# CyrilMorel42/LZ4-JPEG

Measured on AMD Instinct MI355X. Metric: LZ4 compress GB/s + JPEG DCT Mpixel/s at 1/2/4/8 MI355X; % HBM roofline, higher is better.
Workload: dtype u8

## Files before the change

include/lz4r.h:

```cpp
#ifndef LZ4R_H
#define LZ4R_H

#include <stddef.h>
#include <stdint.h>

#ifdef __cplusplus
extern "C" {
#endif

#define LZ4R_BLOCK 300
#define LZ4R_BLOCK_BOUND 1152

#define LZ4R_OK 0
#define LZ4R_ERR_ARG (-1)
#define LZ4R_ERR_TOO_SMALL (-2)
#define LZ4R_ERR_CAPACITY (-3)
#define LZ4R_ERR_HIP (-4)
#define LZ4R_ERR_NOMEM (-5)
#define LZ4R_ERR_CORRUPT (-6)
#define LZ4R_LEN_CORRUPT (1ull << 63)


typedef struct lz4r_ctx lz4r_ctx;

int lz4r_ctx_create(lz4r_ctx **ctx);
void lz4r_ctx_destroy(lz4r_ctx *ctx);

size_t lz4r_compress_bound(size_t n);
size_t lz4r_nblocks(size_t n);

size_t lz4r_launch_chunk_blocks(void);

int lz4r_compress_device(lz4r_ctx *ctx, const void *d_in, size_t n,
                         void *d_out, size_t cap, size_t *out_len,
                         void *stream);

int lz4r_compress_async(lz4r_ctx *ctx, const void *d_in, size_t n,
                        void *d_out, size_t cap, void *d_out_len,
                        void *stream);

int lz4r_compress_segment_async(lz4r_ctx *ctx, const void *d_in, size_t n,
                                void *d_out, size_t cap, void *d_out_len,
                                int final_shard, void *stream);

int lz4r_block_matches_device(const void *d_in, size_t n, void *d_matches, void *stream);

int lz4r_window_matches_device(const void *d_in, size_t n, void *d_matches, void *stream);

int lz4r_copy_block_sizes(const lz4r_ctx *ctx, void *dst, size_t count,
                          void *stream);

int lz4r_copy_block_offsets(const lz4r_ctx *ctx, void *dst, size_t count,
                            void *stream);

int lz4r_block_offsets_device(const lz4r_ctx *ctx, const void **d_offsets,
                              size_t *count);

int lz4r_decompress(const uint8_t *in, size_t in_len, uint8_t *out, size_t cap,
                    size_t *out_len);

int lz4r_decompress_device(const void *d_in, size_t in_len, const void *d_block_offsets,
                           size_t nb, void *d_out, size_t out_cap, void *d_result,
                           void *stream);

int lz4r_decompress_stream_device(const void *d_in, size_t in_len, void *d_out,
                                  size_t out_cap, size_t *out_len, void *stream);

int lz4r_decompress_stream(const uint8_t *in, size_t in_len, uint8_t *out, size_t cap,
                           size_t *out_len);

typedef struct lz4r_read { uint64_t src, len, dst; } lz4r_read;

size_t lz4r_read_items(size_t max_len);

int lz4r_read_device(const void *d_in, size_t in_len, const void *d_block_offsets,
                     size_t nb, const void *d_reads, size_t nreads, size_t max_len,
                     void *d_out, size_t out_cap, void *d_result, void *stream);

int lz4r_stream_index_device(const void *d_in, size_t in_len, void *d_block_offsets,
                             size_t cap_blocks, size_t *nb, size_t *decoded_len, void *stream);

int lz4r_compress(const uint8_t *in, size_t n, uint8_t *out, size_t cap,
                  size_t *out_len);

int lz4r_check(lz4r_ctx *ctx, void *stream);

int lz4r_set_timing(lz4r_ctx *ctx, int enable);
int lz4r_last_timing(lz4r_ctx *ctx, float *ms_call, float *ms_match);
int lz4r_timed_calls(lz4r_ctx *ctx, size_t max, float *ms_call, float *ms_match, size_t *count);

const char *lz4r_strerror(int code);

#ifdef __cplusplus
}
#endif
#endif
```

lz4-jpeg_amd/csrc/lz4r.hip:

```cpp
#include <hip/hip_ext.h>
#include <hip/hip_runtime.h>
#include <limits.h>
#include <stdint.h>
#include <stdio.h>
#include <stdlib.h>
#include <algorithm>
#include <new>
#include <vector>

#include "../../include/lz4r.h"
#include "lz4r_prof.h"
#include "wave64.h"
#include "lz4r_layout.h"
#include "lz4r_tiles.h"
#include "lz4r_matches.h"
#include "lz4r_scan.h"
#include "lz4r_emit.h"

#ifndef LZ4R_CHUNK_LOG2
#define LZ4R_CHUNK_LOG2 24
#endif
constexpr size_t kChunk = size_t(1) << LZ4R_CHUNK_LOG2;
static_assert(kChunk % kPart == 0, "chunks start on a scan partial");
static_assert((kChunk / 8) * 8 * 64 < (size_t(1) << 32), "chunk grid fits HIP's limit");
constexpr size_t kMaxInput = size_t(1) << 40;

struct lz4r_ctx {
  int device = 0;
  size_t cap_blocks = 0;
  size_t cap_slots = 0;
  uint16_t *bsizes = nullptr;
  uint64_t *boff = nullptr;
  uint8_t *slots = nullptr;
  uint32_t *tsz = nullptr;
  uint32_t *gsum = nullptr;
  uint64_t *part = nullptr;
  uint64_t *len = nullptr;
  uint32_t *status = nullptr;
  uint64_t *verdict = nullptr;
  size_t last_nb = 0;
  bool checkable = false;
  struct timed_set {
    hipEvent_t a = nullptr, c = nullptr;
    std::vector<hipEvent_t> tiles;
    size_t chunks = 0;
  };
  std::vector<timed_set> tsets;
  size_t timed_calls = 0;
  bool timing = false;
};
constexpr size_t kTimedCalls = 4096;

namespace {

void free_scratch(lz4r_ctx *c) {
  (void)hipFree(c->bsizes);
  (void)hipFree(c->boff);
  (void)hipFree(c->tsz);
  (void)hipFree(c->gsum);
  (void)hipFree(c->part);
  (void)hipFree(c->slots);
  c->bsizes = nullptr;
  c->boff = nullptr;
  c->slots = nullptr;
  c->tsz = nullptr;
  c->gsum = nullptr;
  c->part = nullptr;
  c->cap_blocks = 0;
  c->cap_slots = 0;
}

int ensure_scratch(lz4r_ctx *c, size_t nb) {
  const size_t need_slots = std::min(nb, kChunk);
  if (nb <= c->cap_blocks && need_slots <= c->cap_slots) return LZ4R_OK;
  free_scratch(c);
  const size_t cap = nb + nb / 8 + 1024;
  const size_t cap_slots = std::min(cap, kChunk);
  const size_t parts = (cap + kPart - 1) / kPart;
  const size_t groups = (cap + kGT - 1) / kGT;
  if (hipMalloc(&c->slots, cap_slots * (size_t)kSlot) != hipSuccess ||
      hipMalloc(&c->bsizes, cap * sizeof(uint16_t)) != hipSuccess ||
      hipMalloc(&c->boff, cap * sizeof(uint64_t)) != hipSuccess ||
      hipMalloc(&c->tsz, cap * sizeof(uint32_t)) != hipSuccess ||
      hipMalloc(&c->gsum, groups * sizeof(uint32_t)) != hipSuccess ||
      hipMalloc(&c->part, parts * sizeof(uint64_t)) != hipSuccess) {
    (void)hipGetLastError();
    free_scratch(c);
    return LZ4R_ERR_NOMEM;
  }
  c->cap_blocks = cap;
  c->cap_slots = cap_slots;
  return LZ4R_OK;
}

int make_event(hipEvent_t *e) {
  return hipEventCreateWithFlags(e, hipEventDisableSystemFence) == hipSuccess ? LZ4R_OK
                                                                               : LZ4R_ERR_HIP;
}

int next_timed_set(lz4r_ctx *c, size_t nchunks, lz4r_ctx::timed_set **out) {
  const size_t i = c->timed_calls % kTimedCalls;
  if (c->tsets.size() <= i) c->tsets.resize(i + 1);
  lz4r_ctx::timed_set &t = c->tsets[i];
  if ((!t.a && make_event(&t.a) != LZ4R_OK) || (!t.c && make_event(&t.c) != LZ4R_OK))
    return LZ4R_ERR_HIP;
  while (t.tiles.size() < 2 * nchunks) {
    hipEvent_t e = nullptr;
    if (make_event(&e) != LZ4R_OK) return LZ4R_ERR_HIP;
    t.tiles.push_back(e);
  }
  t.chunks = nchunks;
  *out = &t;
  return LZ4R_OK;
}

void destroy_events(lz4r_ctx *c) {
  for (auto &t : c->tsets) {
    if (t.a) (void)hipEventDestroy(t.a);
    if (t.c) (void)hipEventDestroy(t.c);
    for (hipEvent_t e : t.tiles) (void)hipEventDestroy(e);
  }
  c->tsets.clear();
}

int timed_ms(const lz4r_ctx::timed_set &t, float *ms_call, float *ms_match) {
  if (hipEventSynchronize(t.c) != hipSuccess) return LZ4R_ERR_HIP;
  float a = 0.f, b = 0.f;
  if (hipEventElapsedTime(&a, t.a, t.c) != hipSuccess) return LZ4R_ERR_HIP;
  for (size_t k = 0; k < t.chunks; ++k) {
    float x = 0.f;
    if (hipEventElapsedTime(&x, k == 0 ? t.a : t.tiles[2 * k], t.tiles[2 * k + 1]) != hipSuccess)
      return LZ4R_ERR_HIP;
    b += x;
  }
  *ms_call = a;
  *ms_match = b;
  return LZ4R_OK;
}

int run(lz4r_ctx *c, const void *d_in, size_t n, void *d_out, size_t cap,
        void *d_len, int hdr, void *stream) {
  if (!c || !d_in || !d_out || !d_len) return LZ4R_ERR_ARG;
  if (hdr && n < (size_t)kBlk) return LZ4R_ERR_TOO_SMALL;
  if (n == 0 || n > kMaxInput) return LZ4R_ERR_ARG;
  const size_t nb = (n + kBlk - 1) / kBlk;
  const size_t nchunks = (nb + kChunk - 1) / kChunk;
  int rc = ensure_scratch(c, nb);
  if (rc != LZ4R_OK) return rc;
  hipStream_t s = static_cast<hipStream_t>(stream);
  const bool timed = c->timing;
  lz4r_ctx::timed_set *ts = nullptr;
  if (timed && (rc = next_timed_set(c, nchunks, &ts)) != LZ4R_OK) return rc;
  auto ev = [&](hipEvent_t e) { return timed ? e : nullptr; };
  const uint8_t *in = static_cast<const uint8_t *>(d_in);
  uint8_t *const ovfs = c->slots + c->cap_slots * (size_t)kHead;
  for (size_t k = 0; k < nchunks; ++k) {
    const size_t b0 = k * kChunk;
    const size_t nbc = std::min(kChunk, nb - b0);
    const size_t b1 = b0 + nbc;
    const uint32_t last_n = (uint32_t)(b1 == nb ? n - (nb - 1) * kBlk : kBlk);
    const uint32_t runs = (uint32_t)((nbc + 8 * kTileRun - 1) / (8 * kTileRun));
    const uint32_t per = runs * kTileRun;
    hipEvent_t t0 = timed ? (k == 0 ? ts->a : ts->tiles[2 * k]) : nullptr;
    hipEvent_t t1 = timed ? ts->tiles[2 * k + 1] : nullptr;
    const auto tiles = ((uintptr_t)in & 3) == 0 ? lz4_tiles<true> : lz4_tiles<false>;
    hipExtLaunchKernelGGL(tiles, dim3(8 * runs), dim3(64), 0, s, t0, t1, 0u, in + b0 * kBlk,
                          (uint32_t)nbc, per, last_n, c->slots, ovfs, c->tsz + b0,
                          c->bsizes + b0, c->status);
    const size_t p0 = b0 / kPart, np = (nbc + kPart - 1) / kPart;
    hipLaunchKernelGGL(lz4_scan_reduce, dim3((unsigned)np), dim3(256), 0, s, c->tsz, b1, p0,
                       c->gsum, c->part);
    hipLaunchKernelGGL(lz4_scan_partials, dim3(1), dim3(1024), 0, s, c->part + p0, np,
                       (uint64_t)hdr, k == 0 ? 1 : 0, k + 1 == nchunks ? 1 : 0, c->status,
                       static_cast<uint64_t *>(d_len), c->verdict);
    const size_t g0 = b0 / kGT, ng = (nbc + kGT - 1) / kGT;
    hipExtLaunchKernelGGL(lz4_emit, dim3((unsigned)(8 * ((ng * kGSplit + 7) / 8))), dim3(64 * kEW), 0, s, nullptr,
                          k + 1 == nchunks ? ev(ts ? ts->c : nullptr) : nullptr, 0u, in,
                          (const uint8_t *)c->slots, (const uint8_t *)ovfs, b0,
                          (const uint32_t *)c->tsz, b1, g0, (const uint32_t *)c->gsum,
                          (const uint64_t *)c->part, static_cast<uint8_t *>(d_out), (uint64_t)cap,
                          hdr, (uint64_t)nb, (uint32_t)(n - (nb - 1) * kBlk), c->boff);
  }
  if (timed) ++c->timed_calls;
  c->last_nb = nb;
  c->checkable = true;
  const hipError_t e = hipGetLastError();
  if (e != hipSuccess && getenv("LZ4R_DEBUG"))
    fprintf(stderr, "lz4r: %s\n", hipGetErrorString(e));
  return e == hipSuccess ? LZ4R_OK : LZ4R_ERR_HIP;
}

int copy_per_block(const lz4r_ctx *c, const void *src, size_t elem, void *dst, size_t count,
                   void *stream) {
  if (!dst || count > c->last_nb) return LZ4R_ERR_ARG;
  if (count == 0) return LZ4R_OK;
  hipStream_t s = static_cast<hipStream_t>(stream);
  if (hipMemcpyAsync(dst, src, count * elem, hipMemcpyDefault, s) != hipSuccess ||
      hipStreamSynchronize(s) != hipSuccess)
    return LZ4R_ERR_HIP;
  return LZ4R_OK;
}

}

extern "C" {

int lz4r_ctx_create(lz4r_ctx **out) {
  if (!out) return LZ4R_ERR_ARG;
  lz4r_ctx *c = new (std::nothrow) lz4r_ctx();
  if (!c) return LZ4R_ERR_NOMEM;
  if (hipGetDevice(&c->device) != hipSuccess ||
      hipMalloc(&c->len, 3 * sizeof(uint64_t)) != hipSuccess ||
      hipMemset(c->len, 0, 3 * sizeof(uint64_t)) != hipSuccess) {
    lz4r_ctx_destroy(c);
    return LZ4R_ERR_HIP;
  }
  c->status = reinterpret_cast<uint32_t *>(c->len + 1);
  c->verdict = c->len + 2;
  *out = c;
  return LZ4R_OK;
}

void lz4r_ctx_destroy(lz4r_ctx *c) {
  if (!c) return;
  free_scratch(c);
  (void)hipFree(c->len);
  destroy_events(c);
  delete c;
}

size_t lz4r_nblocks(size_t n) { return (n + kBlk - 1) / kBlk; }

size_t lz4r_launch_chunk_blocks(void) { return kChunk; }

size_t lz4r_compress_bound(size_t n) { return 1 + lz4r_nblocks(n) * (size_t)LZ4R_BLOCK_BOUND; }

int lz4r_compress_async(lz4r_ctx *c, const void *d_in, size_t n, void *d_out, size_t cap,
                        void *d_len, void *stream) {
  return run(c, d_in, n, d_out, cap, d_len, 1, stream);
}

int lz4r_compress_segment_async(lz4r_ctx *c, const void *d_in, size_t n, void *d_out,
                                size_t cap, void *d_len, int final_shard, void *stream) {
  if (!c || !d_len) return LZ4R_ERR_ARG;
  if (!final_shard && n % kBlk != 0) return LZ4R_ERR_ARG;
  if (n == 0) {
    c->last_nb = 0;
    c->checkable = false;
    hipStream_t s = static_cast<hipStream_t>(stream);
    if (c->timing) {
      lz4r_ctx::timed_set *ts = nullptr;
      const int rc = next_timed_set(c, 0, &ts);
      if (rc != LZ4R_OK) return rc;
      (void)hipEventRecord(ts->a, s);
      (void)hipEventRecord(ts->c, s);
      ++c->timed_calls;
    }
    return hipMemsetAsync(d_len, 0, sizeof(uint64_t), s) == hipSuccess ? LZ4R_OK : LZ4R_ERR_HIP;
  }
  return run(c, d_in, n, d_out, cap, d_len, 0, stream);
}

int lz4r_compress_device(lz4r_ctx *c, const void *d_in, size_t n, void *d_out, size_t cap,
                         size_t *out_len, void *stream) {
  if (!c || !out_len) return LZ4R_ERR_ARG;
  int rc = run(c, d_in, n, d_out, cap, c->len, 1, stream);
  if (rc != LZ4R_OK) return rc;
  uint64_t got = 0;
  hipStream_t s = static_cast<hipStream_t>(stream);
  hipError_t e = hipMemcpyAsync(&got, c->len, sizeof(got), hipMemcpyDeviceToHost, s);
  if (e == hipSuccess) e = hipStreamSynchronize(s);
  if (e != hipSuccess) {
    if (getenv("LZ4R_DEBUG")) fprintf(stderr, "lz4r: %s\n", hipGetErrorString(e));
    return LZ4R_ERR_HIP;
  }
  *out_len = (size_t)(got & ~kLenCorrupt);
  if (got & kLenCorrupt) return LZ4R_ERR_CORRUPT;
  return *out_len > cap ? LZ4R_ERR_CAPACITY : LZ4R_OK;
}

int lz4r_block_matches_device(const void *d_in, size_t n, void *d_matches, void *stream) {
  if (!d_in || !d_matches || n == 0 || n > kMaxInput) return LZ4R_ERR_ARG;
  const size_t nb = (n + kBlk - 1) / kBlk;
  const uint8_t *in = static_cast<const uint8_t *>(d_in);
  uint32_t *mo = static_cast<uint32_t *>(d_matches);
  for (size_t b0 = 0; b0 < nb; b0 += kChunk) {
    const size_t nbc = std::min(kChunk, nb - b0);
    const uint32_t last_n = (uint32_t)(b0 + nbc == nb ? n - (nb - 1) * kBlk : kBlk);
    hipLaunchKernelGGL(lz4_matches, dim3((unsigned)nbc), dim3(64), 0,
                       static_cast<hipStream_t>(stream), in + b0 * kBlk, (uint32_t)nbc, last_n,
                       mo + b0 * kBlk);
  }
  return hipGetLastError() == hipSuccess ? LZ4R_OK : LZ4R_ERR_HIP;
}

int lz4r_window_matches_device(const void *d_in, size_t n, void *d_matches, void *stream) {
  if (!d_in || !d_matches || n == 0 || n > 0xFFFFFFFFull) return LZ4R_ERR_ARG;
  constexpr size_t kPosChunk = size_t(1) << 26;
  for (size_t p0 = 0; p0 < n; p0 += kPosChunk) {
    const size_t np = std::min(kPosChunk, n - p0);
    hipLaunchKernelGGL(lz4_window_matches, dim3((unsigned)((np + 3) / 4)), dim3(256), 0,
                       static_cast<hipStream_t>(stream), static_cast<const uint8_t *>(d_in),
                       (uint32_t)n, (uint32_t)p0, static_cast<uint32_t *>(d_matches));
  }
  return hipGetLastError() == hipSuccess ? LZ4R_OK : LZ4R_ERR_HIP;
}

int lz4r_copy_block_sizes(const lz4r_ctx *c, void *dst, size_t count, void *stream) {
  if (!c) return LZ4R_ERR_ARG;
  return copy_per_block(c, c->bsizes, sizeof(uint16_t), dst, count, stream);
}

int lz4r_copy_block_offsets(const lz4r_ctx *c, void *dst, size_t count, void *stream) {
  if (!c) return LZ4R_ERR_ARG;
  return copy_per_block(c, c->boff, sizeof(uint64_t), dst, count, stream);
}

int lz4r_block_offsets_device(const lz4r_ctx *c, const void **d_offsets, size_t *count) {
  if (!c || !d_offsets || !count) return LZ4R_ERR_ARG;
  *d_offsets = c->boff;
  *count = c->last_nb;
  return LZ4R_OK;
}

int lz4r_compress(const uint8_t *in, size_t n, uint8_t *out, size_t cap, size_t *out_len) {
  if (!in || !out || !out_len) return LZ4R_ERR_ARG;
  if (n < (size_t)kBlk) return LZ4R_ERR_TOO_SMALL;
  lz4r_ctx *c = nullptr;
  int rc = lz4r_ctx_create(&c);
  if (rc != LZ4R_OK) return rc;
  void *din = nullptr, *dout = nullptr;
  const size_t dcap = lz4r_compress_bound(n);
  if (hipMalloc(&din, n + 16) != hipSuccess || hipMalloc(&dout, dcap) != hipSuccess) {
    (void)hipFree(din);
    lz4r_ctx_destroy(c);
    return LZ4R_ERR_NOMEM;
  }
  if (hipMemcpy(din, in, n, hipMemcpyHostToDevice) != hipSuccess) rc = LZ4R_ERR_HIP;
  size_t got = 0;
  if (rc == LZ4R_OK) rc = lz4r_compress_device(c, din, n, dout, dcap, &got, nullptr);
  if (rc == LZ4R_OK) {
    *out_len = got;
    if (got > cap) rc = LZ4R_ERR_CAPACITY;
    else if (hipMemcpy(out, dout, got, hipMemcpyDeviceToHost) != hipSuccess) rc = LZ4R_ERR_HIP;
  }
  (void)hipFree(din);
  (void)hipFree(dout);
  lz4r_ctx_destroy(c);
  return rc;
}

int lz4r_check(lz4r_ctx *c, void *stream) {
  if (!c) return LZ4R_ERR_ARG;
  if (!c->checkable) return LZ4R_OK;
  uint64_t v = 0;
  hipStream_t s = static_cast<hipStream_t>(stream);
  if (hipMemcpyAsync(&v, c->verdict, sizeof(v), hipMemcpyDeviceToHost, s) != hipSuccess ||
      hipStreamSynchronize(s) != hipSuccess)
    return LZ4R_ERR_HIP;
  return v ? LZ4R_ERR_CORRUPT : LZ4R_OK;
}

int lz4r_set_timing(lz4r_ctx *c, int enable) {
  if (!c) return LZ4R_ERR_ARG;
  c->timing = enable != 0;
  if (c->timing) c->timed_calls = 0;
  return LZ4R_OK;
}

int lz4r_last_timing(lz4r_ctx *c, float *ms_call, float *ms_match) {
  if (!c || c->timed_calls == 0) return LZ4R_ERR_ARG;
  float a = 0.f, b = 0.f;
  const int rc = timed_ms(c->tsets[(c->timed_calls - 1) % kTimedCalls], &a, &b);
  if (rc != LZ4R_OK) return rc;
  if (ms_call) *ms_call = a;
  if (ms_match) *ms_match = b;
  return LZ4R_OK;
}

int lz4r_timed_calls(lz4r_ctx *c, size_t max, float *ms_call, float *ms_match, size_t *count) {
  if (!c || !count || (max && (!ms_call || !ms_match))) return LZ4R_ERR_ARG;
  const size_t n = std::min(std::min(c->timed_calls, kTimedCalls), max);
  for (size_t j = 0; j < n; ++j) {
    const size_t i = (c->timed_calls - n + j) % kTimedCalls;
    const int rc = timed_ms(c->tsets[i], &ms_call[j], &ms_match[j]);
    if (rc != LZ4R_OK) return rc;
  }
  *count = n;
  return LZ4R_OK;
}

const char *lz4r_strerror(int code) {
  switch (code) {
    case LZ4R_OK: return "ok";
    case LZ4R_ERR_ARG: return "invalid argument";
    case LZ4R_ERR_TOO_SMALL: return "input shorter than one 300-byte block";
    case LZ4R_ERR_CAPACITY: return "output buffer too small";
    case LZ4R_ERR_HIP: return "HIP runtime error";
    case LZ4R_ERR_NOMEM: return "device allocation failed";
    case LZ4R_ERR_CORRUPT: return "corrupt stream";
    default: return "unknown error";
  }
}

}
```

lz4-jpeg_amd/csrc/lz4r_tiles.h:

```cpp
#pragma once
#include <type_traits>

#include "lz4r_prof.h"
#include "lz4r_tile_lds.h"

namespace {

typedef unsigned int u32x2 __attribute__((ext_vector_type(2)));
typedef unsigned int u32x3 __attribute__((ext_vector_type(3)));
struct TileKeys {
  u32x2 r0;
  u32x3 r[4];
};

__device__ __forceinline__ int block_lane() {
  int lane = threadIdx.x;
  asm volatile("" : "+v"(lane));
  __builtin_assume(lane >= 0 && lane < 64);
  return lane;
}

__device__ __forceinline__ void load_keys(TileKeys &K, const uint8_t *__restrict__ src, int lane) {
  typedef u32x2 u32x2_a4 __attribute__((aligned(4)));
  typedef u32x3 u32x3_a4 __attribute__((aligned(4)));
  const uint32_t *bw = reinterpret_cast<const uint32_t *>(src) + (lane >> 2);
  K.r0 = *reinterpret_cast<const u32x2_a4 *>(bw);
#pragma unroll
  for (int r = 1; r < 5; ++r) K.r[r - 1] = *reinterpret_cast<const u32x3_a4 *>(bw + 16 * r - 1);
}

__device__ __forceinline__ void keys_arrived(TileKeys &K) {
  asm volatile("" : "+v"(K.r0), "+v"(K.r[0]), "+v"(K.r[1]), "+v"(K.r[2]), "+v"(K.r[3]));
}

struct RecBatch {
  uint32_t seqv = 0;
  uint32_t p0 = 0;
};
constexpr int kHalf = 32;

__device__ __forceinline__ uint32_t half_incl_add(uint32_t v) {
  v += dpp<0x111, 0xf, 0xf>(v);
  v += dpp<0x112, 0xf, 0xf>(v);
  v += dpp<0x114, 0xf, 0xf>(v);
  v += dpp<0x118, 0xf, 0xf>(v);
  v += dpp<0x142, 0xa, 0xf>(v);
  return v;
}

__device__ __forceinline__ void store_block_totals(uint64_t m, uint32_t tb, int lane, uint32_t hdr,
                                                   uint32_t w, uint8_t *heads, uint32_t *usz,
                                                   uint16_t *bsizes) {
  const uint32_t bl = tb + (uint32_t)lane;
  uint64_t save;
  asm volatile(
      "s_and_saveexec_b64 %0, %1\n\t"
      "global_store_dword %2, %5, %7\n\t"
      "global_store_dword %3, %6, %8\n\t"
      "global_store_short %4, %6, %9\n\t"
      "s_or_b64 exec, exec, %0"
      : "=&s"(save)
      : "s"(m), "v"(bl * (uint32_t)kHead), "v"(bl * 4u), "v"(bl * 2u), "v"(hdr), "v"(w), "s"(heads),
        "s"(usz), "s"(bsizes)
      : "memory", "scc");
}

template <bool kFast>
__device__ __forceinline__ void flush_records(const uint32_t wv, const uint32_t f0,
                                              const uint32_t f1, const uint32_t tb,
                                              uint8_t *__restrict__ heads,
                                              uint8_t *__restrict__ ovfs,
                                              uint32_t *__restrict__ usz,
                                              uint16_t *__restrict__ bsizes, const int lane) {
  constexpr int n = kBlk;
  const int M = (int)((wv >> 9) & 255u);
  const int end = (int)(wv >> 19);
  const uint32_t cq = (uint32_t)(end - M);
  const uint32_t upv = dpp<0x138, 0xf, 0xf>((uint32_t)end);
  const int pend = (int)sel_mask(0x0000000100000001ull, 0u, upv);
  const int L = (int)cq - pend;
  const uint64_t am = (((1ull << f0) - 1ull) | ((1ull << f1) - 1ull) << kHalf) & ballot(pend < n);
  uint32_t ws;
  if constexpr (kFast) {
    ws = (uint32_t)(L + 5) + (L >= 15 ? 1u : 0u) + (L == 270 ? 1u : 0u) + (M >= 19 ? 1u : 0u);
  } else {
    ws = (uint32_t)(L + 5 + (L >= 15 ? 1 : 0) + (L == 270 ? 1 : 0)) * 0x10001u;
    ws += M >= 19 ? 0x10001u : 0u;
    ws += (uint32_t)(M - 1) < 3u ? 0x10000u : 0u;
  }
  const uint32_t sc = half_incl_add(sel_mask(am, ws, 0u));
  const uint32_t t0 = (uint32_t)__builtin_amdgcn_readlane((int)sc, kHalf - 1);
  const uint32_t t1 = lane63(sc);
  const uint32_t ns0 = (uint32_t)__popc((uint32_t)am), ns1 = (uint32_t)__popc((uint32_t)(am >> kHalf));
  uint32_t hdr, wb;
  if constexpr (kFast) {
    hdr = write_lane<0>(t1 | (ns1 << 16), t0 | (ns0 << 16));
    wb = (hdr & 0xFFFFu) + 3u;
  } else {
    uint32_t z0 = t0 >> 16, z1 = t1 >> 16;
    asm("" : "+s"(z0));
    asm("" : "+s"(z1));
    hdr = write_lane<0>(z1 | (ns1 << 16), z0 | (ns0 << 16));
    wb = write_lane<0>((t1 & 0xFFFFu) + 3u, (t0 & 0xFFFFu) + 3u);
  }
  constexpr uint64_t kHeadLanes = ((1ull << (kHeadW - 1)) - 1ull) * 0x0000000100000001ull;
  const uint32_t x4 = 4u * (uint32_t)lane, h32 = (uint32_t)lane & (uint32_t)kHalf;
  store_lanes1(am & kHeadLanes, reinterpret_cast<uint32_t *>(heads + (size_t)tb * kHead),
               x4 - h32 * ((128 - kHead) / kHalf), wv);
  const uint64_t om = am & ~kHeadLanes;
  if (om)
    store_lanes1(om, reinterpret_cast<uint32_t *>(ovfs + (size_t)tb * kOvf) - kHeadW,
                 x4 + (h32 << 3) + (h32 >> 1), wv);
  static_assert(kOvf - 4 * kHalf == 8 * kHalf + kHalf / 2, "the second overflow slot from lane & 32");
  store_block_totals(f1 ? 3ull : 1ull, tb, lane, hdr, wb, heads, usz, bsizes);
}
static_assert((128 - kHead) % kHalf == 0 && kHeadW - 1 < kHalf, "the second half's records");

template <bool kMatchesOnly, bool kFull>
__device__ __forceinline__ void encode_block(TileLds &S, int n_arg, const uint8_t *__restrict__ gsrc,
                                            TileKeys &K, const uint8_t *__restrict__ next,
                                            uint32_t *__restrict__ mout,
                                            uint8_t *__restrict__ heads,
                                            uint8_t *__restrict__ ovfs,
                                            uint32_t *__restrict__ status, const int lane,
                                            ProfClock &prof, RecBatch &B, const bool flush_after,
                                            uint32_t *__restrict__ usz,
                                            uint16_t *__restrict__ bsizes, const uint32_t t) {
  const int n = kFull ? kBlk : n_arg;
  constexpr int base = kInOff;

  const int nk = n >= 4 ? n - 3 : 0;

  bool walk[5];
  uint32_t qn = 0;
  uint32_t key[5];
  {
    const uint32_t sh = (uint32_t)lane & 3u;
    const uint32_t *bw = reinterpret_cast<const uint32_t *>(S.buf) + (kInOff >> 2) + (lane >> 2);
    uint32_t pt[5], adr[5], set[5];
    const uint32_t dummy = (uint32_t)(kRecOff + 4 * (192 + lane) - kHeadOff);
#pragma unroll
    for (int r = 0; r < 5; ++r) {
      const uint32_t w1 = !kFull ? bw[16 * r] : r ? K.r[r ? r - 1 : 0].y : K.r0.x;
      const uint32_t w2 = !kFull ? bw[16 * r + 1] : r ? K.r[r ? r - 1 : 0].z : K.r0.y;
      key[r] = __builtin_amdgcn_alignbyte(w2, w1, sh);
      const uint32_t hv = key[r] * 2654435761u;
      if (r == 0) {
        const uint32_t pb = (uint32_t)__builtin_amdgcn_update_dpp(0, (int)key[0], 0x138, 0xf,
                                                                 0xf, false);
        pt[0] = __builtin_amdgcn_perm(pb, key[0], 0x00040C0Cu);
      } else {
        const uint32_t w0 = kFull ? K.r[r - 1].x : bw[16 * r - 1];
        pt[r] = __builtin_amdgcn_perm(w1, w0, 0x04030C0Cu + sh * 0x01010000u);
      }
      const int p = 64 * r + lane;
      const bool act = (kFull && r < 4) || p < nk;
// ... 164 lines not shown

  PROF_MARK(4);
  const uint32_t lim = (uint32_t)(4 * n + 1) << 17;
  auto walk_words = [&](uint32_t &sq, int l0) {
    int l1 = l0;
    if (w0 < lim) {
      static_assert(kWordOff < 65536, "ds_read offset field");
      uint32_t w = w0, va = w0 >> 17, vt;
      asm volatile(
          "s_mov_b32 m0, %7\n"
          "1:\n\t"
          "v_writelane_b32 %0, %1, m0\n\t"
          "ds_read_b32 %3, %2 offset:%c6\n\t"
          "s_add_u32 m0, m0, 1\n\t"
          "s_waitcnt lgkmcnt(0)\n\t"
          "v_readfirstlane_b32 %1, %3\n\t"
          "v_lshrrev_b32 %2, 17, %3\n\t"
          "s_cmp_lt_u32 %1, %5\n\t"
          "s_cbranch_scc1 1b\n\t"
          "s_mov_b32 %4, m0"
          : "+v"(sq), "+s"(w), "+v"(va), "=&v"(vt), "=&s"(l1)
          : "s"(lim), "i"(kWordOff), "s"(l0)
          : "scc", "memory");
    }
    return l1;
  };
  constexpr bool kBat = kFull && kTileRun > 1;
  int it;
  uint32_t seqv;
  if constexpr (kBat) {
    const uint32_t p0 = B.p0;
    const int l0 = (int)(p0 >> 16);
    const uint32_t before = B.seqv;
    seqv = before;
    __builtin_amdgcn_s_setprio(3);
    const int l1 = walk_words(seqv, l0);
    __builtin_amdgcn_s_setprio(0);
    it = l1 - l0;
    const bool fits = it < kHalf;
    PROF_MARK(5);
    keys_arrived(K);
    PROF_MARK(7);
    uint32_t f0 = p0 & 255u, f1 = 0u, slowm = p0 & 256u, rv = before;
    if (fits) {
      rv = (lane == l1) ? (uint32_t)n << 19 : seqv;
      slowm |= fastw ? 0u : 256u;
      if (l0 == 0) {
        if (!flush_after) {
          B.seqv = rv;
          B.p0 = (uint32_t)(it + 1) | slowm | (uint32_t)kHalf << 16;
          return;
        }
        f0 = (uint32_t)(it + 1);
      } else {
        f1 = (uint32_t)(it + 1);
      }
    }
    B.p0 = 0;
    if (f0) {
      const uint32_t tb = t - (uint32_t)(l0 >> 5);
      if (slowm == 0u)
        flush_records<true>(rv, f0, f1, tb, heads, ovfs, usz, bsizes, lane);
      else
        flush_records<false>(rv, f0, f1, tb, heads, ovfs, usz, bsizes, lane);
    }
    PROF_MARK(6);
    if (fits) return;
    seqv = 0;
    walk_words(seqv, 0);
  } else {
    seqv = 0;
    __builtin_amdgcn_s_setprio(3);
    it = walk_words(seqv, 0);
    __builtin_amdgcn_s_setprio(0);
  }
  const bool slow = it > 64;
  int Sv_slow = 0;
  if (slow) {
    const uint8_t *const wb = reinterpret_cast<const uint8_t *>(S.word);
    for (uint32_t w = w0; w < lim;
         w = (uint32_t)__builtin_amdgcn_readfirstlane(
             (int)*reinterpret_cast<const uint32_t *>(wb + (w >> 17)))) {
      if (lane == 0) S.seq()[Sv_slow] = w;
      ++Sv_slow;
    }
    wave_sync();
  }
  PROF_MARK(5);
  uint32_t *const head = reinterpret_cast<uint32_t *>(heads + (size_t)t * kHead);
  uint32_t *const ovf = reinterpret_cast<uint32_t *>(ovfs + (size_t)t * kOvf);
  int nseq = 0;
  int ocar = 3;
  int szsum = 0;
  int end_prev = 0;
  auto round = [&](auto fast, int s0, uint32_t wv) {
    const int kk = s0 + lane;
    const int M = (int)((wv >> 9) & 255u);
    const int end = (int)(wv >> 19);
    const uint32_t cq = (uint32_t)(end - M);
    const uint64_t ismm = ballot((int)cq < n);
    const int nm_r = __popcll(ismm);
    const uint32_t upv = dpp<0x138, 0xf, 0xf>((uint32_t)end);
    const int pend = lane == 0 ? end_prev : (int)upv;
    end_prev = (int)lane63((uint32_t)end);
    const int L = (int)cq - pend;
    const uint64_t am = ismm | (ballot(lane == nm_r) & ballot(pend < n));
    if constexpr (decltype(fast)::value) {
      const uint32_t ws = (uint32_t)(L + 5) + (L >= 15 ? 1u : 0u) + (L == 270 ? 1u : 0u) +
                          (M >= 19 ? 1u : 0u);
      const uint32_t tot = lane63(wave_incl_add(sel_mask(am, ws, 0u)));
      ocar += (int)tot;
      szsum += (int)tot;
    } else {
      uint32_t ws = (uint32_t)(L + 5 + (L >= 15 ? 1 : 0) + (L == 270 ? 1 : 0)) * 0x10001u;
      ws += M >= 19 ? 0x10001u : 0u;
      ws += (uint32_t)(M - 1) < 3u ? 0x10000u : 0u;
      const uint32_t tot = lane63(wave_incl_add(sel_mask(am, ws, 0u)));
      ocar += (int)(tot & 0xFFFFu);
      szsum += (int)(tot >> 16);
    }
    if (s0 == 0) {
      store_lanes1(am & ((1ull << (kHeadW - 1)) - 1), head, 4u * (uint32_t)kk, wv);
      if (am >> (kHeadW - 1)) store_lanes1(am >> (kHeadW - 1) << (kHeadW - 1), ovf - kHeadW,
                                           4u * (uint32_t)kk, wv);
    } else {
      store_lanes1(am, ovf - kHeadW, 4u * (uint32_t)kk, wv);
    }
    nseq += (int)__popcll(am);
    return nm_r == 64;
  };
  {
    const uint32_t wtail = (uint32_t)n << 19;
    const uint32_t c0 = slow ? S.seq()[lane] : (lane < it ? seqv : wtail);
    auto rounds = [&](auto fast) {
      if (round(fast, 0, c0)) {
        for (int s0 = 64;; s0 += 64) {
          const int kk = s0 + lane;
          if (!round(fast, s0, slow && kk < Sv_slow ? S.seq()[kk] : wtail)) break;
        }
      }
    };
    if (fastw)
      rounds(std::true_type{});
    else
      rounds(std::false_type{});
  }
  PROF_MARK(6);
  store_block_totals(1ull, t, lane, (uint32_t)szsum | ((uint32_t)nseq << 16), (uint32_t)ocar, heads,
                     usz, bsizes);
}

template <bool kAligned>
__global__ __launch_bounds__(64) __attribute__((amdgpu_waves_per_eu(8, 8))) void lz4_tiles(
    const uint8_t *__restrict__ in, uint32_t nb, uint32_t per, uint32_t last_n,
    uint8_t *__restrict__ heads, uint8_t *__restrict__ ovfs, uint32_t *__restrict__ usz,
    uint16_t *__restrict__ bsizes, uint32_t *__restrict__ status) {
  __shared__ TileLds S;
  ProfClock prof = PROF_START();
  const uint32_t t0 = (blockIdx.x & 7u) * per + (blockIdx.x >> 3) * (uint32_t)kTileRun;
  if (t0 >= nb) return;
  const uint32_t t1 = kTileRun == 1 ? t0 + 1 : min(t0 + (uint32_t)kTileRun, nb);
  const uint32_t nbg = nb + (last_n >= 24 ? 1u : 0u);
  auto full = [&](uint32_t t) { return kAligned && t + 2 < nbg; };
  TileKeys K;
  RecBatch B;
  const uint8_t *src = in + (size_t)t0 * kBlk;
  for (uint32_t t = t0; t < t1; ++t, src += kBlk) {
    const int lane = block_lane();
    const int n = t + 1 + (last_n >= 24 ? 1u : 0u) == nbg ? (int)last_n : kBlk;
    if (full(t)) {
      if (t == t0) {
        load_keys(K, src, lane);
        keys_arrived(K);
        PROF_MARK(7);
      }
      const bool pf = kTileRun > 1 && t + 1 < t1 && full(t + 1);
      encode_block<false, true>(S, kBlk, src, K, pf ? src + kBlk : src, nullptr, heads, ovfs,
                                status, lane, prof, B, !pf, usz, bsizes, t);
    } else {
      for (int i = lane; i < n; i += 64) S.buf[kInOff + i] = src[i];
      if (lane < 16) S.buf[kInOff + n + lane] = 0;
      wave_sync();
      if (t == t0) PROF_MARK(7);
      encode_block<false, false>(S, n, nullptr, K, nullptr, nullptr, heads, ovfs, status, lane,
                                 prof, B, true, usz, bsizes, t);
    }
    wave_sync();
  }
  PROF_FLUSH();
}

}
```

lz4-jpeg_amd/lz4jpeg/_lib.py:

```python
import ctypes
import os

_HERE = os.path.dirname(os.path.abspath(__file__))
LIB_PATH = os.environ.get("LZ4JPEG_LIB") or os.path.join(_HERE, "liblz4jpeg.so")

_c_size = ctypes.c_size_t
_vp = ctypes.c_void_p
_i = ctypes.c_int

SIGNATURES = [
    ("lz4r_ctx_create", _i, [ctypes.POINTER(_vp)]),
    ("lz4r_ctx_destroy", None, [_vp]),
    ("lz4r_compress_bound", _c_size, [_c_size]),
    ("lz4r_nblocks", _c_size, [_c_size]),
    ("lz4r_launch_chunk_blocks", _c_size, []),
    ("lz4r_compress_device", _i, [_vp, _vp, _c_size, _vp, _c_size, ctypes.POINTER(_c_size), _vp]),
    ("lz4r_compress_async", _i, [_vp, _vp, _c_size, _vp, _c_size, _vp, _vp]),
    ("lz4r_compress_segment_async", _i, [_vp, _vp, _c_size, _vp, _c_size, _vp, _i, _vp]),
    ("lz4r_copy_block_sizes", _i, [_vp, _vp, _c_size, _vp]),
    ("lz4r_copy_block_offsets", _i, [_vp, _vp, _c_size, _vp]),
    ("lz4r_block_offsets_device", _i, [_vp, ctypes.POINTER(_vp), ctypes.POINTER(_c_size)]),
    ("lz4r_block_matches_device", _i, [_vp, _c_size, _vp, _vp]),
    ("lz4r_window_matches_device", _i, [_vp, _c_size, _vp, _vp]),
    ("lz4r_compress", _i, [_vp, _c_size, _vp, _c_size, ctypes.POINTER(_c_size)]),
    ("lz4r_decompress", _i, [_vp, _c_size, _vp, _c_size, ctypes.POINTER(_c_size)]),
    ("lz4r_decompress_device", _i, [_vp, _c_size, _vp, _c_size, _vp, _c_size, _vp, _vp]),
    ("lz4r_decompress_stream_device", _i, [_vp, _c_size, _vp, _c_size, ctypes.POINTER(_c_size),
                                           _vp]),
    ("lz4r_decompress_stream", _i, [_vp, _c_size, _vp, _c_size, ctypes.POINTER(_c_size)]),
    ("lz4r_read_items", _c_size, [_c_size]),
    ("lz4r_read_device", _i, [_vp, _c_size, _vp, _c_size, _vp, _c_size, _c_size, _vp, _c_size,
                              _vp, _vp]),
    ("lz4r_stream_index_device", _i, [_vp, _c_size, _vp, _c_size, ctypes.POINTER(_c_size),
                                      ctypes.POINTER(_c_size), _vp]),
    ("lz4r_check", _i, [_vp, _vp]),
    ("lz4r_set_timing", _i, [_vp, _i]),
    ("lz4r_last_timing", _i, [_vp, ctypes.POINTER(ctypes.c_float), ctypes.POINTER(ctypes.c_float)]),
    ("lz4r_timed_calls", _i, [_vp, _c_size, ctypes.POINTER(ctypes.c_float),
                              ctypes.POINTER(ctypes.c_float), ctypes.POINTER(_c_size)]),
    ("lz4r_strerror", ctypes.c_char_p, [_i]),
    ("jpegr_coef_count", _c_size, [_i, _i]),
    ("jpegr_encode_device", _i, [_vp, _i, _i, _i, _vp, _vp]),
    ("jpegr_dct_raw_device", _i, [_vp, _i, _i, _i, _vp, _vp]),
    ("jpegr_encode", _i, [_vp, _i, _i, _vp]),
    ("jpegr_time_device", _i, [_vp, _i, _i, _i, _vp, _i, _vp, ctypes.POINTER(ctypes.c_float)]),
    ("jpegr_reconstruct_device", _i, [_vp, _vp, _i, _i, _i, _vp, _vp]),
    ("jpegr_entropy_scratch_bytes", _c_size, [_c_size]),
    ("jpegr_entropy_encode_device", _i, [_vp, _c_size, _vp, _vp, _vp, _vp, _vp, _vp]),
    ("jpegr_entropy_decode_device", _i, [_vp, _vp, _vp, _c_size, _vp, _vp, _vp]),
    ("jpegr_pack_bound", _c_size, [_i, _i, _i]),
    ("jpegr_pack_scratch_bytes", _c_size, [_c_size]),
    ("jpegr_pack_device", _i, [_vp, _vp, _vp, _i, _i, _i, _vp, _c_size, _vp, _vp, _vp]),
    ("jpegr_stream_info", _i, [_vp, ctypes.POINTER(_i), ctypes.POINTER(_i), ctypes.POINTER(_i)]),
    ("jpegr_unpack_device", _i, [_vp, _c_size, _i, _i, _i, _vp, _vp, _vp, _vp, _vp, _vp]),
    ("jpegr_stream_decode_device", _i, [_vp, _c_size, _i, _i, _i, _c_size, _c_size, _vp, _vp, _vp,
                                        _vp]),
    ("jpegr_pack_tight_device", _i, [_vp, _vp, _vp, _i, _i, _i, _vp, _c_size, _vp, _vp, _vp]),
    ("jpegr_stream_format", _i, [_vp, ctypes.POINTER(_i), ctypes.POINTER(_i), ctypes.POINTER(_i),
                                 ctypes.POINTER(_i)]),
    ("jpegr_stream_encode_scratch_bytes", _c_size, [_c_size, _c_size]),
    ("jpegr_stream_encode_device", _i, [_vp, _i, _i, _i, _i, _vp, _c_size, _vp, _vp, _vp, _vp]),
    ("jpegr_stream_index_device", _i, [_vp, _c_size, _i, _i, _i, _vp, _vp, _vp, _vp]),
    ("jpegr_crop_items", _c_size, [_i, _i]),
    ("jpegr_crop_scratch_bytes", _c_size, [_c_size, _i, _i]),
    ("jpegr_crop_device", _i, [_vp, _c_size, _i, _i, _i, _vp, _vp, _c_size, _i, _i, _vp, _c_size,
                               _vp, _vp, _vp]),
    ("jpegr_planes_device", _i, [_vp, _i, _i, _vp, _vp, _vp, _vp]),
    ("jpegr_dct_blocks_device", _i, [_vp, _i, _i, _i, _vp, _vp]),
    ("jpegr_quantize_device", _i, [_vp, _vp, _i, _c_size, _vp]),
    ("jpegr_permute_device", _i, [_vp, _vp, _vp, _i, _c_size, _vp]),
    ("jpegr_strerror", ctypes.c_char_p, [_i]),
    ("lz4jpeg_rand_rgba", None, [ctypes.c_uint, _i, _i, _vp]),
    ("lz4jpeg_random_passages", _c_size, [_vp, _c_size, ctypes.c_uint, _c_size, _c_size, _c_size,
                                         _vp]),
    ("lz4jpeg_rand_rgba_stream", None, [ctypes.c_uint, ctypes.c_uint64, _c_size, _vp]),
    ("lz4jpeg_rand_states", None, [ctypes.c_uint, ctypes.c_uint64, ctypes.c_uint64, _c_size,
                                   _vp]),
    ("lz4jpeg_passage_starts", _c_size, [_c_size, ctypes.c_uint, _c_size, ctypes.c_uint64,
                                         _c_size, _vp]),
    ("lz4jpeg_rand_rgba_device", _i, [ctypes.c_uint, ctypes.c_uint64, _c_size, _vp, _vp]),
    ("lz4jpeg_random_passages_device", _i, [_vp, _c_size, ctypes.c_uint, _c_size,
                                            ctypes.c_uint64, _c_size, _vp, _vp]),
    ("lz4_encode", None, []),
    ("find_longest_match", ctypes.c_uint8, [_vp, _c_size, ctypes.POINTER(ctypes.c_uint16)]),
    ("block_encode", None, [_vp, _c_size, _vp, _vp, _vp, _vp]),
    ("write_output", None, [_vp, _vp]),
    ("LZ4_decode", None, [ctypes.c_char_p, ctypes.c_char_p]),
    ("discrete_cosine_transform", None, [_vp, _c_size, _c_size, ctypes.POINTER(ctypes.POINTER(
        ctypes.c_double))]),
    ("Quantize", None, [ctypes.POINTER(ctypes.POINTER(ctypes.c_double)), _vp, _c_size]),
    ("zigzag_pattern", None, [_c_size, _c_size, _vp, _vp]),
]

_lib = None


class LibraryMissing(RuntimeError):
    pass


def lib():
    global _lib
    if _lib is not None:
        return _lib
    if not os.path.exists(LIB_PATH):
        raise LibraryMissing(
            f"{LIB_PATH} not built: run `make -C {os.path.dirname(os.path.dirname(_HERE))}` "
            "(the HIP path is the only compute path; there is no CPU fallback)")
    handle = ctypes.CDLL(LIB_PATH)
    for name, res, args in SIGNATURES:
        fn = getattr(handle, name)
        fn.restype = res
        fn.argtypes = args
    _lib = handle
    return _lib


class Lz4Error(RuntimeError):
    def __init__(self, code, where=""):
        msg = lib().lz4r_strerror(code).decode()
        super().__init__(f"{where}: lz4r error {code} ({msg})")
        self.code = code


class JpegError(RuntimeError):
    def __init__(self, code, where=""):
        msg = lib().jpegr_strerror(code).decode()
        super().__init__(f"{where}: jpegr error {code} ({msg})")
        self.code = code


LZ4R_OK = 0
LZ4R_ERR_ARG = -1
LZ4R_ERR_TOO_SMALL = -2
LZ4R_ERR_CAPACITY = -3
LZ4R_ERR_HIP = -4
LZ4R_ERR_NOMEM = -5
LZ4R_ERR_CORRUPT = -6
LZ4R_BLOCK = 300
LZ4R_BLOCK_BOUND = 1152
```

lz4-jpeg_amd/lz4jpeg/lz4.py:

```python
import ctypes

import numpy as np

from . import _lib
from ._lib import Lz4Error, LZ4R_BLOCK, LZ4R_BLOCK_BOUND

BLOCK = LZ4R_BLOCK


class InputTooSmall(Lz4Error):
    pass


def _raise(code, where):
    if code == _lib.LZ4R_ERR_TOO_SMALL:
        raise InputTooSmall(code, where)
    raise Lz4Error(code, where)


def nblocks(n):
    return (n + BLOCK - 1) // BLOCK


def compress_bound(n):
    return int(_lib.lib().lz4r_compress_bound(n))


def _stream_handle(stream=None):
    import torch
    s = stream if stream is not None else torch.cuda.current_stream()
    return ctypes.c_void_p(s.cuda_stream)


class Compressor:

    def __init__(self):
        L = _lib.lib()
        h = ctypes.c_void_p()
        rc = L.lz4r_ctx_create(ctypes.byref(h))
        if rc != 0:
            _raise(rc, "lz4r_ctx_create")
        self._h = h

    def close(self):
        if getattr(self, "_h", None):
            _lib.lib().lz4r_ctx_destroy(self._h)
            self._h = None

    def __del__(self):
        try:
            self.close()
        except Exception:
            pass

    def compress_device(self, d_in, n=None, d_out=None, stream=None):
        import torch
        n = d_in.numel() if n is None else n
        if d_out is None:
            d_out = torch.empty(compress_bound(n), dtype=torch.uint8, device=d_in.device)
        got = ctypes.c_size_t(0)
        rc = _lib.lib().lz4r_compress_device(self._h, ctypes.c_void_p(d_in.data_ptr()), n,
                                             ctypes.c_void_p(d_out.data_ptr()), d_out.numel(),
                                             ctypes.byref(got), _stream_handle(stream))
        if rc != 0:
            _raise(rc, "lz4r_compress_device")
        return d_out, got.value

    def compress_async(self, d_in, n, d_out, d_len, stream=None, segment=False,
                       final_shard=None):
        if segment and final_shard is None:
            raise ValueError("compress_async(segment=True) needs final_shard=True/False")
        L = _lib.lib()
        args = (self._h, ctypes.c_void_p(d_in.data_ptr()), n, ctypes.c_void_p(d_out.data_ptr()),
                d_out.numel(), ctypes.c_void_p(d_len.data_ptr()))
        if segment:
            rc = L.lz4r_compress_segment_async(*args, 1 if final_shard else 0,
                                               _stream_handle(stream))
        else:
            rc = L.lz4r_compress_async(*args, _stream_handle(stream))
        if rc != 0:
            _raise(rc, "lz4r_compress_segment_async" if segment else "lz4r_compress_async")

    @staticmethod
    def async_length(d_len):
        v = int(d_len.item())
        if v < 0:
            raise Lz4Error(_lib.LZ4R_ERR_CORRUPT,
                           "lz4r_compress_*_async: corrupt LDS index (LZ4R_LEN_CORRUPT)")
        return v

    def block_offsets(self, count, stream=None):
        out = np.empty(count, dtype=np.uint64)
        rc = _lib.lib().lz4r_copy_block_offsets(self._h, out.ctypes.data_as(ctypes.c_void_p),
                                                count, _stream_handle(stream))
        if rc != 0:
            _raise(rc, "lz4r_copy_block_offsets")
        return out

    def block_offsets_device(self):
        ptr, cnt = ctypes.c_void_p(), ctypes.c_size_t(0)
        rc = _lib.lib().lz4r_block_offsets_device(self._h, ctypes.byref(ptr), ctypes.byref(cnt))
        if rc != 0:
            _raise(rc, "lz4r_block_offsets_device")
        return ptr.value, cnt.value

    def check(self, stream=None):
        rc = _lib.lib().lz4r_check(self._h, _stream_handle(stream))
        if rc != 0:
            _raise(rc, "lz4r_check")

    def set_timing(self, enable=True):
        _lib.lib().lz4r_set_timing(self._h, 1 if enable else 0)

    def last_timing(self):
        a, b = ctypes.c_float(0), ctypes.c_float(0)
        rc = _lib.lib().lz4r_last_timing(self._h, ctypes.byref(a), ctypes.byref(b))
        if rc != 0:
            _raise(rc, "lz4r_last_timing")
        return a.value, b.value

    def timed_calls(self, max_calls=4096):
        a = (ctypes.c_float * max_calls)()
        b = (ctypes.c_float * max_calls)()
        cnt = ctypes.c_size_t(0)
        rc = _lib.lib().lz4r_timed_calls(self._h, max_calls, a, b, ctypes.byref(cnt))
        if rc != 0:
            _raise(rc, "lz4r_timed_calls")
        return list(a[:cnt.value]), list(b[:cnt.value])

    def compress(self, data):
        import torch
        buf = np.frombuffer(bytes(data), dtype=np.uint8)
        if buf.size < BLOCK:
            raise InputTooSmall(_lib.LZ4R_ERR_TOO_SMALL, "compress")
        d_in = torch.from_numpy(buf.copy()).cuda()
        d_out, length = self.compress_device(d_in)
        torch.cuda.synchronize()
        return d_out[:length].cpu().numpy().tobytes()


def compress(data):
    buf = np.frombuffer(bytes(data), dtype=np.uint8)
    n = buf.size
    if n < BLOCK:
        raise InputTooSmall(_lib.LZ4R_ERR_TOO_SMALL, "lz4r_compress")
    cap = 1 + nblocks(n) * LZ4R_BLOCK_BOUND
    out = np.empty(cap, dtype=np.uint8)
    got = ctypes.c_size_t(0)
    rc = _lib.lib().lz4r_compress(buf.ctypes.data_as(ctypes.c_void_p), n,
                                  out.ctypes.data_as(ctypes.c_void_p), cap, ctypes.byref(got))
    if rc != 0:
        _raise(rc, "lz4r_compress")
    return out[:got.value].tobytes()


def decompress(stream, cap=None):
    buf = np.frombuffer(bytes(stream), dtype=np.uint8)
    if cap is None:
        cap = (buf.size // 5 + 1) * BLOCK
    out = np.empty(max(cap, 1), dtype=np.uint8)
    got = ctypes.c_size_t(0)
    rc = _lib.lib().lz4r_decompress(buf.ctypes.data_as(ctypes.c_void_p), buf.size,
                                    out.ctypes.data_as(ctypes.c_void_p), cap, ctypes.byref(got))
    if rc != 0:
        _raise(rc, "lz4r_decompress")
    return out[:got.value].tobytes()


def decompress_device(d_stream, length, d_offsets, nb, out_cap, d_out=None, stream=None,
                      check=True):
    import torch
    if d_out is None:
        d_out = torch.empty(max(out_cap, 1), dtype=torch.uint8, device=d_stream.device)
    res = torch.empty(2, dtype=torch.int64, device=d_stream.device)
    offs = d_offsets if isinstance(d_offsets, int) else d_offsets.data_ptr()
    rc = _lib.lib().lz4r_decompress_device(
        ctypes.c_void_p(d_stream.data_ptr()), length, ctypes.c_void_p(offs), nb,
        ctypes.c_void_p(d_out.data_ptr()), out_cap, ctypes.c_void_p(res.data_ptr()),
        _stream_handle(stream))
    if rc != 0:
        _raise(rc, "lz4r_decompress_device")
    if not check:
        return d_out, None
    if stream is not None:
        stream.synchronize()
    n, bad = (int(x) for x in res.cpu().tolist())
    if bad != -1:
        raise Lz4Error(_lib.LZ4R_ERR_CORRUPT, f"lz4r_decompress_device: block {bad - 1}")
    if n > out_cap:
        raise Lz4Error(_lib.LZ4R_ERR_CAPACITY,
                       f"lz4r_decompress_device: needs {n} bytes, capacity {out_cap}")
    return d_out, n


def decompress_stream_device(d_stream, length, out_cap, d_out=None, stream=None):
    import torch
    if d_out is None:
        d_out = torch.empty(max(out_cap, 1), dtype=torch.uint8, device=d_stream.device)
    got = ctypes.c_size_t(0)
    rc = _lib.lib().lz4r_decompress_stream_device(
        ctypes.c_void_p(d_stream.data_ptr()), length, ctypes.c_void_p(d_out.data_ptr()), out_cap,
        ctypes.byref(got), _stream_handle(stream))
    if rc != 0:
        _raise(rc, "lz4r_decompress_stream_device")
    return d_out, got.value


def decompress_stream(stream_bytes, cap=None):
    buf = np.frombuffer(bytes(stream_bytes), dtype=np.uint8)
    if cap is None:
        cap = (buf.size // 8 + 1) * BLOCK
    out = np.empty(max(cap, 1), dtype=np.uint8)
    got = ctypes.c_size_t(0)
    rc = _lib.lib().lz4r_decompress_stream(buf.ctypes.data_as(ctypes.c_void_p), buf.size,
                                           out.ctypes.data_as(ctypes.c_void_p), cap,
                                           ctypes.byref(got))
    if rc != 0:
        _raise(rc, "lz4r_decompress_stream")
    return out[:got.value].tobytes()


def stream_index_device(d_stream, length, stream=None):
    import torch
    cap = length // 64 + 64
    for _ in range(2):
        d_offs = torch.empty(cap, dtype=torch.int64, device=d_stream.device)
        nb, n = ctypes.c_size_t(0), ctypes.c_size_t(0)
        rc = _lib.lib().lz4r_stream_index_device(
            ctypes.c_void_p(d_stream.data_ptr()), length, ctypes.c_void_p(d_offs.data_ptr()), cap,
            ctypes.byref(nb), ctypes.byref(n), _stream_handle(stream))
        if rc != _lib.LZ4R_ERR_CAPACITY:
            break
        cap = nb.value
    if rc != 0:
        _raise(rc, "lz4r_stream_index_device")
    return d_offs[:nb.value], nb.value, n.value


def read_items(max_len):
    return int(_lib.lib().lz4r_read_items(max_len))


def read_device(d_stream, length, d_offsets, nb, d_src, d_len, max_len, d_dst=None, d_out=None,
                out_cap=None, stream=None, check=True):
    import torch
    nreads = d_src.numel()
    if d_dst is None:
        d_dst = torch.cumsum(d_len, 0) - d_len
    if out_cap is None:
        if d_out is not None:
            out_cap = d_out.numel()
        elif check and nreads:
            out_cap = int((d_dst + d_len).max().item())
        else:
            out_cap = nreads * max_len
    if d_out is None:
        d_out = torch.empty(max(out_cap, 1), dtype=torch.uint8, device=d_stream.device)
    if nreads == 0:
        return d_out, d_dst, (0 if check else None)
    d_reads = torch.stack((d_src, d_len, d_dst), dim=1).contiguous()
    res = torch.empty(2, dtype=torch.int64, device=d_stream.device)
    offs = d_offsets if isinstance(d_offsets, int) else d_offsets.data_ptr()
    rc = _lib.lib().lz4r_read_device(
        ctypes.c_void_p(d_stream.data_ptr()), length, ctypes.c_void_p(offs), nb,
        ctypes.c_void_p(d_reads.data_ptr()), nreads, max_len, ctypes.c_void_p(d_out.data_ptr()),
# ... 57 lines not shown
```

Baseline: 467.4.

## Taper tile-run lengths at the grid tail to balance workgroup load

Replaces the uniform per-workgroup tile run with a tapered schedule. Most workgroups take full kTileRun runs, and a final set of S workgroups per section takes halved, quartered, and smaller runs. The goal is to shrink the tail where a few long-running workgroups finish last while the GPU sits idle. The default is 1024 taper workgroups, and a new API exposes the count. This adds more workgroups and some index arithmetic per launch.

Result: no change. 472.0, median of 6 (+1.0%).

```diff
diff --git a/include/lz4r.h b/include/lz4r.h
--- a/include/lz4r.h
+++ b/include/lz4r.h
@@ -89,6 +89,8 @@
 int lz4r_last_timing(lz4r_ctx *ctx, float *ms_call, float *ms_match);
 int lz4r_timed_calls(lz4r_ctx *ctx, size_t max, float *ms_call, float *ms_match, size_t *count);
 
+int lz4r_set_taper(lz4r_ctx *ctx, size_t workgroups);
+
 const char *lz4r_strerror(int code);
 
 #ifdef __cplusplus
diff --git a/lz4-jpeg_amd/csrc/lz4r.hip b/lz4-jpeg_amd/csrc/lz4r.hip
--- a/lz4-jpeg_amd/csrc/lz4r.hip
+++ b/lz4-jpeg_amd/csrc/lz4r.hip
@@ -22,7 +22,7 @@
 #endif
 constexpr size_t kChunk = size_t(1) << LZ4R_CHUNK_LOG2;
 static_assert(kChunk % kPart == 0, "chunks start on a scan partial");
-static_assert((kChunk / 8) * 8 * 64 < (size_t(1) << 32), "chunk grid fits HIP's limit");
+static_assert((kChunk / 8) * 8 * 64 < (size_t(1) << 31), "chunk grid fits HIP's limit");
 constexpr size_t kMaxInput = size_t(1) << 40;
 
 struct lz4r_ctx {
@@ -38,6 +38,7 @@
   uint64_t *len = nullptr;
   uint32_t *status = nullptr;
   uint64_t *verdict = nullptr;
+  uint32_t taper = kTaperDefault;
   size_t last_nb = 0;
   bool checkable = false;
   struct timed_set {
@@ -159,14 +160,13 @@
     const size_t nbc = std::min(kChunk, nb - b0);
     const size_t b1 = b0 + nbc;
     const uint32_t last_n = (uint32_t)(b1 == nb ? n - (nb - 1) * kBlk : kBlk);
-    const uint32_t runs = (uint32_t)((nbc + 8 * kTileRun - 1) / (8 * kTileRun));
-    const uint32_t per = runs * kTileRun;
+    const TileGrid grid = tile_grid((uint32_t)nbc, c->taper);
     hipEvent_t t0 = timed ? (k == 0 ? ts->a : ts->tiles[2 * k]) : nullptr;
     hipEvent_t t1 = timed ? ts->tiles[2 * k + 1] : nullptr;
     const auto tiles = ((uintptr_t)in & 3) == 0 ? lz4_tiles<true> : lz4_tiles<false>;
-    hipExtLaunchKernelGGL(tiles, dim3(8 * runs), dim3(64), 0, s, t0, t1, 0u, in + b0 * kBlk,
-                          (uint32_t)nbc, per, last_n, c->slots, ovfs, c->tsz + b0,
-                          c->bsizes + b0, c->status);
+    hipExtLaunchKernelGGL(tiles, dim3(8 * grid.wgs), dim3(64), 0, s, t0, t1, 0u, in + b0 * kBlk,
+                          (uint32_t)nbc, grid.per, grid.taper, last_n, c->slots, ovfs,
+                          c->tsz + b0, c->bsizes + b0, c->status);
     const size_t p0 = b0 / kPart, np = (nbc + kPart - 1) / kPart;
     hipLaunchKernelGGL(lz4_scan_reduce, dim3((unsigned)np), dim3(256), 0, s, c->tsz, b1, p0,
                        c->gsum, c->part);
@@ -368,6 +368,12 @@
   return LZ4R_OK;
 }
 
+int lz4r_set_taper(lz4r_ctx *c, size_t workgroups) {
+  if (!c || workgroups > (size_t(1) << 20)) return LZ4R_ERR_ARG;
+  c->taper = (uint32_t)workgroups;
+  return LZ4R_OK;
+}
+
 int lz4r_last_timing(lz4r_ctx *c, float *ms_call, float *ms_match) {
   if (!c || c->timed_calls == 0) return LZ4R_ERR_ARG;
   float a = 0.f, b = 0.f;
diff --git a/lz4-jpeg_amd/csrc/lz4r_tile_grid.h b/lz4-jpeg_amd/csrc/lz4r_tile_grid.h
--- /dev/null
+++ b/lz4-jpeg_amd/csrc/lz4r_tile_grid.h
@@ -0,0 +1,69 @@
+#pragma once
+#include <stdint.h>
+
+#include "lz4r_layout.h"
+
+#if defined(__HIPCC__)
+#define LZ4R_GRID_FN __host__ __device__ __forceinline__
+#else
+#define LZ4R_GRID_FN inline
+#endif
+
+namespace {
+
+#ifndef LZ4R_TAPER_MIN
+#define LZ4R_TAPER_MIN 2
+#endif
+constexpr int kTaperMin = LZ4R_TAPER_MIN;
+static_assert(kTaperMin >= 1 && (kTaperMin & (kTaperMin - 1)) == 0, "the taper's shortest run");
+
+constexpr int taper_sections() {
+  int n = 0;
+  if ((kTileRun & (kTileRun - 1)) == 0)
+    for (int l = kTileRun / 2; l >= kTaperMin; l /= 2) ++n;
+  return n;
+}
+constexpr int kTaperSecs = taper_sections();
+constexpr uint32_t kTaperBlocks = (uint32_t)(kTileRun - (kTileRun >> kTaperSecs));
+constexpr uint32_t kTaperDefault = 1024;
+
+struct TileGrid {
+  uint32_t per;
+  uint32_t wgs;
+  uint32_t taper;
+};
+
+inline TileGrid tile_grid(uint32_t nb, uint32_t S) {
+  const uint32_t q = (nb + 7) / 8;
+  const uint64_t T = (uint64_t)S * kTaperBlocks;
+  TileGrid g;
+  if (T != 0 && (uint64_t)q >= 4 * T) {
+    const uint32_t bulk = (q - (uint32_t)T + kTileRun - 1) / kTileRun;
+    g.per = bulk * kTileRun + (uint32_t)T;
+    g.wgs = bulk + (uint32_t)kTaperSecs * S;
+    g.taper = S;
+  } else {
+    g.wgs = (q + kTileRun - 1) / kTileRun;
+    g.per = g.wgs * kTileRun;
+    g.taper = 0;
+  }
+  return g;
+}
+
+LZ4R_GRID_FN void tile_run(uint32_t i, uint32_t per, uint32_t S, uint32_t &first, uint32_t &len) {
+  first = i * (uint32_t)kTileRun;
+  len = (uint32_t)kTileRun;
+  if (kTaperSecs == 0 || S == 0) return;
+  const uint32_t bulk = (per - S * kTaperBlocks) / (uint32_t)kTileRun;
+  if (i < bulk) return;
+  uint32_t j = i - bulk;
+  len = (uint32_t)kTileRun / 2;
+  for (int s = 1; s < kTaperSecs; ++s)
+    if (j >= S) {
+      j -= S;
+      len >>= 1;
+    }
+  first = bulk * (uint32_t)kTileRun + S * ((uint32_t)kTileRun - 2 * len) + j * len;
+}
+
+}
diff --git a/lz4-jpeg_amd/csrc/lz4r_tiles.h b/lz4-jpeg_amd/csrc/lz4r_tiles.h
--- a/lz4-jpeg_amd/csrc/lz4r_tiles.h
+++ b/lz4-jpeg_amd/csrc/lz4r_tiles.h
@@ -2,6 +2,7 @@
 #include <type_traits>
 
 #include "lz4r_prof.h"
+#include "lz4r_tile_grid.h"
 #include "lz4r_tile_lds.h"
 
 namespace {
@@ -472,14 +473,16 @@
 
 template <bool kAligned>
 __global__ __launch_bounds__(64) __attribute__((amdgpu_waves_per_eu(8, 8))) void lz4_tiles(
-    const uint8_t *__restrict__ in, uint32_t nb, uint32_t per, uint32_t last_n,
+    const uint8_t *__restrict__ in, uint32_t nb, uint32_t per, uint32_t taper, uint32_t last_n,
     uint8_t *__restrict__ heads, uint8_t *__restrict__ ovfs, uint32_t *__restrict__ usz,
     uint16_t *__restrict__ bsizes, uint32_t *__restrict__ status) {
   __shared__ TileLds S;
   ProfClock prof = PROF_START();
-  const uint32_t t0 = (blockIdx.x & 7u) * per + (blockIdx.x >> 3) * (uint32_t)kTileRun;
+  uint32_t first, len;
+  tile_run(blockIdx.x >> 3, per, taper, first, len);
+  const uint32_t t0 = (blockIdx.x & 7u) * per + first;
   if (t0 >= nb) return;
-  const uint32_t t1 = kTileRun == 1 ? t0 + 1 : min(t0 + (uint32_t)kTileRun, nb);
+  const uint32_t t1 = min(t0 + len, nb);
   const uint32_t nbg = nb + (last_n >= 24 ? 1u : 0u);
   auto full = [&](uint32_t t) { return kAligned && t + 2 < nbg; };
   TileKeys K;
diff --git a/lz4-jpeg_amd/lz4jpeg/_lib.py b/lz4-jpeg_amd/lz4jpeg/_lib.py
--- a/lz4-jpeg_amd/lz4jpeg/_lib.py
+++ b/lz4-jpeg_amd/lz4jpeg/_lib.py
@@ -38,6 +38,7 @@
     ("lz4r_last_timing", _i, [_vp, ctypes.POINTER(ctypes.c_float), ctypes.POINTER(ctypes.c_float)]),
     ("lz4r_timed_calls", _i, [_vp, _c_size, ctypes.POINTER(ctypes.c_float),
                               ctypes.POINTER(ctypes.c_float), ctypes.POINTER(_c_size)]),
+    ("lz4r_set_taper", _i, [_vp, _c_size]),
     ("lz4r_strerror", ctypes.c_char_p, [_i]),
     ("jpegr_coef_count", _c_size, [_i, _i]),
     ("jpegr_encode_device", _i, [_vp, _i, _i, _i, _vp, _vp]),
diff --git a/lz4-jpeg_amd/lz4jpeg/lz4.py b/lz4-jpeg_amd/lz4jpeg/lz4.py
--- a/lz4-jpeg_amd/lz4jpeg/lz4.py
+++ b/lz4-jpeg_amd/lz4jpeg/lz4.py
@@ -111,6 +111,11 @@
 
     def set_timing(self, enable=True):
         _lib.lib().lz4r_set_timing(self._h, 1 if enable else 0)
+
+    def set_taper(self, workgroups):
+        rc = _lib.lib().lz4r_set_taper(self._h, workgroups)
+        if rc != 0:
+            _raise(rc, "lz4r_set_taper")
 
     def last_timing(self):
         a, b = ctypes.c_float(0), ctypes.c_float(0)
```
